# javieryu/nn_distributed_training

Hardware: NVIDIA H100
Metric: consensus node-rounds/sec (DiNNO, dist_mnist_PAPER; rounds/sec x graph nodes) (higher is better)
Workload: dtype fp64

## Files before the change

### nn_distributed_training_b200/ops/csrc/bindings.cpp

```cpp
#include <torch/extension.h>
#include <cstring>
#include <string>
#include <ATen/cuda/CUDAContext.h>
#include <pybind11/pybind11.h>

#include "consensus.h"
#include "mnist.h"

namespace py = pybind11;
using namespace nndt;

static inline cudaStream_t cur_stream() { return at::cuda::getCurrentCUDAStream().stream(); }
static inline void check(cudaError_t e, const char* what) {
  if (e != cudaSuccess) throw std::runtime_error(std::string(what) + ": " + cudaGetErrorString(e));
}
template <typename P> static P* ptr(const py::dict& d, const char* k) {
  if (!d.contains(k) || d[k].is_none()) return nullptr;
  return reinterpret_cast<P*>(d[k].cast<uint64_t>());
}
static int geti(const py::dict& d, const char* k, int dflt = 0) { return d.contains(k) ? d[k].cast<int>() : dflt; }
static double getf(const py::dict& d, const char* k, double dflt = 0) { return d.contains(k) ? d[k].cast<double>() : dflt; }

struct MnistOp {
  mnist::Args a{};
// ... 62 lines not shown
  c.nbr_rank = ptr<const int>(d, "nbr_rank"); c.dmax = geti(d, "dmax");
  c.rdr_deg = ptr<const int>(d, "rdr_deg"); c.rdr_rank = ptr<const int>(d, "rdr_rank"); c.rmax = geti(d, "rmax", 1);
  c.round_ctr = ptr<int>(d, "round_ctr");
  c.rho = ptr<const T>(d, "rho"); c.lr = ptr<const T>(d, "lr"); c.alpha = ptr<const T>(d, "alpha");
  c.graph_id = ptr<const int>(d, "graph_id");
  c.calls = ptr<int>(d, "calls");
  c.loss_part = ptr<const float>(d, "loss_part"); c.tloss = ptr<float>(d, "tloss");
  c.tdecay = (float)getf(d, "tdecay", 0.0); c.loss_S = geti(d, "loss_S", 1);
  c.flags = ptr<int>(d, "flags"); c.peer_flag = ptr<const int64_t>(d, "peer_flag");
  c.world = geti(d, "world", 1); c.rank = geti(d, "rank", 0);
  c.done_ctr = ptr<unsigned int>(d, "done_ctr"); c.err = ptr<int>(d, "err");
  c.notify_mask = d.contains("notify_mask") ? d["notify_mask"].cast<unsigned long long>() : ~0ull;
  c.node_order = ptr<const int>(d, "node_order");
  c.timeline = ptr<long long>(d, "timeline");
  c.pub_seq = ptr<int>(d, "pub_seq"); c.nbr_seq = ptr<const int64_t>(d, "nbr_seq");
  c.sum_mode = geti(d, "sum_mode", 0); c.n_total = geti(d, "n_total", 0);
  c.sum_local = ptr<double>(d, "sum_local"); c.sum_mc = ptr<const double>(d, "sum_mc");
  c.sum_flags = ptr<int>(d, "sum_flags"); c.peer_sum_flag = ptr<const int64_t>(d, "peer_sum_flag");
  return c;
}

template <typename T>
struct ConsensusOp {
  consensus::Common<T> c{};
  consensus::DinnoArgs<T> dn{};
  consensus::DsgtArgs<T> gt{};
  consensus::EdArgs<T> ed{};
  consensus::ChocoArgs<T> ch{};
  consensus::SgpArgs<T> sg{};
  explicit ConsensusOp(const py::dict& d) {
    c = common_from<T>(d);
    dn.c = c; gt.c = c; ed.c = c; ch.c = c; sg.c = c;
    sg.x = ptr<T>(d, "x"); sg.w = ptr<double>(d, "w");
    sg.row_stride = d.contains("row_stride") ? d["row_stride"].cast<long long>() : 0;
    ed.psi = ptr<T>(d, "psi");
    ch.x_hat = ptr<T>(d, "x_hat"); ch.s = ptr<T>(d, "s"); ch.live = ptr<const unsigned>(d, "live");
    ch.gamma = (T)getf(d, "gamma", 1.0); ch.code = geti(d, "code", 0);
    ch.code_stride = d.contains("code_stride") ? d["code_stride"].cast<long long>() : 0;
    dn.dual = ptr<T>(d, "dual"); dn.delta = ptr<T>(d, "delta"); dn.m = ptr<T>(d, "m"); dn.v = ptr<T>(d, "v");
    dn.pits = geti(d, "pits", 1); dn.opt = geti(d, "opt", 1); dn.persistent = geti(d, "persistent", 0);
    gt.g_old = ptr<T>(d, "g_old");
    gt.alpha_row = ptr<const T>(d, "alpha_row"); gt.own_tracker = geti(d, "own_tracker", 0);
  }
  void dinno_update(int step) {
    dn.step = step;
    check(consensus::launch_dinno_update<T>(dn, cur_stream()), "dinno_update");
  }
  void local_sum() { check(consensus::launch_local_sum<T>(c, cur_stream()), "local_sum"); }
  void dsgd_mix() { check(consensus::launch_dsgd_mix<T>(c, cur_stream()), "dsgd_mix"); }
  void dsgd_step() { check(consensus::launch_dsgd_step<T>(c, cur_stream()), "dsgd_step"); }
  void dsgt_init() { check(consensus::launch_dsgt_init<T>(gt, cur_stream()), "dsgt_init"); }
  void dsgt_mix() { check(consensus::launch_dsgt_mix<T>(gt, cur_stream()), "dsgt_mix"); }
  void dsgt_track() { check(consensus::launch_dsgt_track<T>(gt, cur_stream()), "dsgt_track"); }
  void ed_mix() { check(consensus::launch_ed_mix<T>(ed, cur_stream()), "ed_mix"); }
  void ed_step() {
    if (ed.psi == nullptr) throw std::runtime_error("ed_step needs the Exact Diffusion row `psi`");
    check(consensus::launch_ed_step<T>(ed, cur_stream()), "ed_step");
  }
  void choco_check(const char* what) const {
    if (ch.x_hat == nullptr || ch.s == nullptr || ch.live == nullptr || ch.code_stride <= 0)
      throw std::runtime_error(std::string(what) + " needs the CHOCO rows `x_hat`, `s`, the `live` mask and `code_stride`");
  }
  void choco_mix() {
    choco_check("choco_mix");
    check(consensus::launch_choco_mix<T>(ch, cur_stream()), "choco_mix");
  }
  void choco_step() {
    choco_check("choco_step");
    check(consensus::launch_choco_step<T>(ch, cur_stream()), "choco_step");
  }
  void sgp_check(const char* what) const {
    if (sg.x == nullptr || sg.w == nullptr || sg.row_stride <= 0)
      throw std::runtime_error(std::string(what) + " needs the SGP rows `x`, `w` and `row_stride`");
  }
  void sgp_mix() {
    sgp_check("sgp_mix");
    check(consensus::launch_sgp_mix<T>(sg, cur_stream()), "sgp_mix");
  }
  void sgp_step() {
    sgp_check("sgp_step");
    check(consensus::launch_sgp_step<T>(sg, cur_stream()), "sgp_step");
  }
};

template <typename T>
struct LocalStepOp {
  consensus::LocalArgs<T> a{};
  explicit LocalStepOp(const py::dict& d) {
    a.c = common_from<T>(d);
    if (a.c.calls == nullptr) throw std::runtime_error("local_step needs the per-node step counter `calls`");
    a.m = ptr<T>(d, "m"); a.v = ptr<T>(d, "v");
    a.budget = ptr<const int>(d, "budget"); a.arrive = ptr<unsigned int>(d, "arrive");
    a.lr = (T)getf(d, "local_lr"); a.opt = geti(d, "opt", 1);
    if (a.budget == nullptr || a.arrive == nullptr) throw std::runtime_error("local_step needs `budget` and `arrive`");
    if (a.opt != consensus::kSGD && (a.m == nullptr || a.v == nullptr))
      throw std::runtime_error("local_step with Adam / AdamW needs the moment rows `m` and `v`");
  }
  void step() { check(consensus::launch_local_step<T>(a, cur_stream()), "local_step"); }
};

template <typename T>
static void bind_consensus(py::module& m, const char* name) {
  py::class_<ConsensusOp<T>>(m, name)
      .def(py::init<const py::dict&>())
      .def("dinno_update", &ConsensusOp<T>::dinno_update)
      .def("local_sum", &ConsensusOp<T>::local_sum)
      .def("dsgd_mix", &ConsensusOp<T>::dsgd_mix)
      .def("dsgd_step", &ConsensusOp<T>::dsgd_step)
      .def("dsgt_init", &ConsensusOp<T>::dsgt_init)
      .def("dsgt_mix", &ConsensusOp<T>::dsgt_mix)
      .def("dsgt_track", &ConsensusOp<T>::dsgt_track)
      .def("ed_mix", &ConsensusOp<T>::ed_mix)
      .def("ed_step", &ConsensusOp<T>::ed_step)
      .def("choco_mix", &ConsensusOp<T>::choco_mix)
      .def("choco_step", &ConsensusOp<T>::choco_step)
      .def("sgp_mix", &ConsensusOp<T>::sgp_mix)
      .def("sgp_step", &ConsensusOp<T>::sgp_step);
}

void bind_mlp(py::module& m);
void bind_rl(py::module& m);
void bind_runtime(py::module& m);

PYBIND11_MODULE(_C, m) {
  m.doc() = "nn_distributed_training_b200 sm_90a kernels";
  py::class_<MnistOp>(m, "MnistOp")
      .def(py::init<const py::dict&>())
      .def("update", &MnistOp::update)
      .def("train", &MnistOp::train)
      .def("eval", &MnistOp::eval);
  py::class_<GatherOp>(m, "GatherOp").def(py::init<const py::dict&>()).def("launch", &GatherOp::launch);
  m.def("debug_batch_indices", [](int mm, int B, int call, int seed, int node, uint64_t out, uint64_t out_size) {
    check(mnist::launch_batch_indices(mm, B, call, seed, node, reinterpret_cast<int*>(out),
                                      reinterpret_cast<int*>(out_size), cur_stream()), "batch_indices");
  });
  m.def("consensus_metric", [](bool f64, uint64_t rows, int N, int n_pad, int local0, int L, uint64_t inv_norm,
                               uint64_t out_pair, uint64_t out_mean) {
    auto r = reinterpret_cast<const int64_t*>(rows);
    auto a = reinterpret_cast<double*>(inv_norm); auto b = reinterpret_cast<double*>(out_pair); auto c = reinterpret_cast<double*>(out_mean);
    check(f64 ? consensus::launch_consensus_metric<double>(r, N, n_pad, local0, L, a, b, c, cur_stream())
              : consensus::launch_consensus_metric<float>(r, N, n_pad, local0, L, a, b, c, cur_stream()), "consensus_metric");
  });
  m.def("convnet_generic_smem_bytes", [](int F, int KS, int LW, int dtype64, int spb) {
    return (size_t)mnist::generic_smem_bytes(mnist::GenericShape{F, KS, LW, dtype64, 0.0, 1.0}, dtype64, spb);
  });
  m.def("make_w1_tensor_map", [](uint64_t theta, int n_pad, int L, int off_w1) {
    unsigned char buf[128];
    check(mnist::make_w1_tensor_map(reinterpret_cast<const float*>(theta), n_pad, L, off_w1, buf), "make_w1_tensor_map");
    return py::bytes(reinterpret_cast<const char*>(buf), 128);
  });
  m.def("mnist_tc_max_clusters", []() { return mnist::tc_max_active_clusters(); });
  m.def("mnist_cl64_max_clusters", [](int nsplit) { return mnist::cl64_max_active_clusters(nsplit); }, py::arg("nsplit") = 1);
  m.def("mnist_cl64_cluster_ctas", []() { return mnist::cl64_cluster_ctas(); });
  m.def("rank_barrier", [](uint64_t slots, uint64_t peer_slot, int world, int rank, int epoch, uint64_t gate, uint64_t err) {
    check(consensus::launch_rank_barrier(reinterpret_cast<int*>(slots), reinterpret_cast<const int64_t*>(peer_slot), world, rank,
                                         epoch, reinterpret_cast<const volatile int*>(gate), reinterpret_cast<int*>(err), cur_stream()),
          "rank_barrier");
  });
  m.def("spin", [](long long cycles) { check(consensus::launch_spin(cycles, cur_stream()), "spin"); });
  bind_consensus<float>(m, "ConsensusOpF32");
  bind_consensus<double>(m, "ConsensusOpF64");
  py::class_<LocalStepOp<float>>(m, "LocalStepOpF32").def(py::init<const py::dict&>()).def("step", &LocalStepOp<float>::step);
  py::class_<LocalStepOp<double>>(m, "LocalStepOpF64").def(py::init<const py::dict&>()).def("step", &LocalStepOp<double>::step);
  bind_mlp(m);
  bind_rl(m);
  bind_runtime(m);
}
```

### nn_distributed_training_b200/ops/csrc/mnist.h

```cpp
#pragma once
#include <cuda_runtime.h>
#include <stdint.h>

namespace nndt {
namespace mnist {

struct Args {
  const float* theta;
  int n_pad, L;
  int off_wc, off_bc, off_w1, off_b1, off_w2, off_b2;
  const void* x;
  const int64_t* y;
  int x_is_u8;
  float mean, inv_std;
  int direct, batch, seed, node0;
  const int* direct_bs;
  const int* shard_off;
  const int* shard_len;
  int* calls;
  unsigned int* arrive;
  int tune;
  long long* prof;
  float* grad_part;
  float* loss_part;
  float* loss_mirror;
  int n_val;
  float* val_loss;
  unsigned char* val_correct;
};

struct GatherArgs {
  const unsigned char* x_host;
  const int64_t* y_host;
  int row_bytes;
  unsigned char* x_stage;
  int64_t* y_stage;
  int* bs_stage;
  int P, L, batch, seed, node0;
  const int* shard_off; const int* shard_len;
  const int* calls0;
  int* stage_round;
  unsigned int* done_ctr;
  int max_blocks;
};
struct GenericShape { int F, KS, LW, dtype64; double mean, inv_std; };
size_t generic_smem_bytes(const GenericShape& gs, int dtype64, int spb);
cudaError_t launch_generic_train(const Args& a, const GenericShape& gs, int spb, int S, cudaStream_t st);
cudaError_t launch_generic_eval(const Args& a, const GenericShape& gs, int ctas_per_node, cudaStream_t st);
cudaError_t make_w1_tensor_map(const float* theta, int n_pad, int L, int off_w1, void* out_map128);
cudaError_t launch_train_tc(const Args& a, const void* w1_map128, int nsplit, cudaStream_t st);
int tc_max_active_clusters();
cudaError_t launch_train_cl64(const Args& a, const GenericShape& gs, int nsplit, cudaStream_t st);
int cl64_max_active_clusters(int nsplit);
int cl64_cluster_ctas();
cudaError_t launch_gather(const GatherArgs& a, cudaStream_t st);
cudaError_t launch_train(const Args& a, int spb, int S, cudaStream_t st);
cudaError_t launch_eval(const Args& a, int ctas_per_node, cudaStream_t st);
cudaError_t launch_batch_indices(int m, int B, int call, int seed, int node, int* out, int* out_size, cudaStream_t st);

}
}
```

### nn_distributed_training_b200/ops/csrc/mnist_cl64.cu

```cuda
#include "mnist_device.cuh"

namespace nndt {
namespace mnist {

namespace cl64 {

constexpr int NT = 512, CL = 4, CELLS = 36, KC = 108, WS = 116, HS = 68;
constexpr int PXR = 10 * HW;
constexpr int KT = (KC + 7) / 8;
constexpr int HR = 68;
NNDT_DEVINL int hr(int j) { return (j >> 4) * 17 + (j & 15); }
constexpr int PART_WC = 0, PART_BC = 75, PART_B1 = 78, PART_W2 = 142, PART_B2 = 782, PART_LOSS = 792, PART_N = 793;

template <int MS>
struct Smem {
  static constexpr int NO = MS / CL;
  static constexpr bool kDoublePix = MS <= 32;
  static constexpr int PXS = kDoublePix ? PXR + 2 : PXR;
  double w[HID * WS];
  double a[MS * WS];
  double h[MS * HS];
  alignas(16) unsigned char img[kDoublePix ? MS * PXS * 8 : MS * PXS];
  double lut[kDoublePix ? 1 : 256];
  double h_loc[NO * HR > CL * 80 ? NO * HR : CL * 80];
  double dh_loc[NO * HID];
  double part[800];
  double w2[NCLS * HR];
  alignas(16) double b1[HID];
  alignas(16) double b2[16];
  double wc[80];
  double dz[NO * 16];
  double red[NO];
  int sidx[MS];
  int label[MS];
  float valid[MS];
  unsigned char arg[MS * KC];
};
static_assert(sizeof(Smem<16>) <= 227 * 1024 && sizeof(Smem<32>) <= 227 * 1024 && sizeof(Smem<64>) <= 227 * 1024,
              "shared memory budget");

NNDT_DEVINL double wmax(double v) {
#pragma unroll
  for (int o = 16; o > 0; o >>= 1) v = fmax(v, __shfl_xor_sync(0xffffffffu, v, o));
  return v;
}
template <int H>
NNDT_DEVINL void fold_half(double (&v)[16], int lane) {
  const bool up = (lane & (2 * H)) != 0;
#pragma unroll
  for (int i = 0; i < H; ++i) {
    const double send = up ? v[i] : v[i + H], keep = up ? v[i + H] : v[i];
    v[i] = keep + __shfl_xor_sync(0xffffffffu, send, 2 * H);
  }
}
NNDT_DEVINL void warp_reduce_scatter16(double (&v)[16], int lane) {
  fold_half<8>(v, lane); fold_half<4>(v, lane); fold_half<2>(v, lane); fold_half<1>(v, lane);
  v[0] += __shfl_xor_sync(0xffffffffu, v[0], 1);
}
NNDT_DEVINL void dmma_nv(double (&c)[4], double a0, double a1, double b) {
  asm("mma.sync.aligned.m16n8k4.row.col.f64.f64.f64.f64 {%0,%1,%2,%3}, {%4,%5}, {%6}, {%0,%1,%2,%3};"
      : "+d"(c[0]), "+d"(c[1]), "+d"(c[2]), "+d"(c[3])
      : "d"(a0), "d"(a1), "d"(b));
}
template <int NJ, int K, class FA, class FB>
NNDT_DEVINL void gemm_k(double (&c)[NJ][4], int m0, int n0, int lane, FA A, FB B) {
  static_assert(K % 4 == 0, "k steps of 4");
  const int g = lane >> 2, t = lane & 3;
  double a0 = A(m0 + g, t), a1 = A(m0 + g + 8, t), b[NJ];
#pragma unroll
  for (int j = 0; j < NJ; ++j) b[j] = B(t, n0 + 8 * j + g);
#pragma unroll
  for (int k0 = 0; k0 < K; k0 += 4) {
    double na0 = 0.0, na1 = 0.0, nb[NJ];
    if (k0 + 4 < K) {
      const int k = k0 + 4 + t;
      na0 = A(m0 + g, k); na1 = A(m0 + g + 8, k);
#pragma unroll
      for (int j = 0; j < NJ; ++j) nb[j] = B(k, n0 + 8 * j + g);
    }
#pragma unroll
    for (int j = 0; j < NJ; ++j) dmma_nv(c[j], a0, a1, b[j]);
    if (k0 + 4 < K) {
      a0 = na0; a1 = na1;
#pragma unroll
      for (int j = 0; j < NJ; ++j) b[j] = nb[j];
    }
  }
}
NNDT_DEVINL void stamp(long long* prof, int idx, int tid) {
  if (prof != nullptr && tid == 0) {
    long long t;
    asm volatile("mov.u64 %0, %%globaltimer;" : "=l"(t));
    prof[idx] = t;
  }
}

template <int MS>
__global__ void __cluster_dims__(CL, 1, 1) __launch_bounds__(NT, 1)
mnist_cl64_train_kernel(const Args a, const GenericShape gs) {
  using SM = Smem<MS>;
  constexpr int NO = SM::NO, PXS = SM::PXS;
  constexpr bool kDoublePix = SM::kDoublePix;
  static_assert(MS % 16 == 0 && NO <= NT / 32, "tile geometry");
  static_assert(CELLS % 2 == 0 && NCLS % 2 == 0 && 32 + NCLS / 2 <= NT, "16-byte parameter copies");
  extern __shared__ __align__(16) unsigned char smem_raw[];
  SM& sm = *reinterpret_cast<SM*>(smem_raw);
  const int tid = threadIdx.x, warp = tid >> 5, lane = tid & 31;
  const int l = blockIdx.z, bsplit = blockIdx.y, nsplit = gridDim.y;
  const int c = (int)cluster_rank();
  const double* th = reinterpret_cast<const double*>(a.theta) + (size_t)l * a.n_pad;
  const double pmean = gs.mean, pis = gs.inv_std;
  const bool u8 = a.x_is_u8 != 0;
  double* imgd = reinterpret_cast<double*>(sm.img);
  auto pix = [&](int s, int p) -> double {
    if constexpr (kDoublePix) return imgd[s * PXS + p];
    else if (u8) return sm.lut[sm.img[s * PXR + p]];
    else return (double)__ldg(reinterpret_cast<const float*>(a.x) + (size_t)sm.sidx[s] * 784 + 6 * HW * c + p);
  };
  long long* prof = a.prof != nullptr ? a.prof + ((l * nsplit + bsplit) * CL + c) * 64 : nullptr;
  stamp(prof, 0, tid);

  const int call = a.calls != nullptr ? a.calls[l] : 0;
  const BatchGeom bg = batch_geom<true>(a, l, call);
  if (tid < MS) {
    int idx = 0, lab = 0; float ok = 0.f;
    const uint32_t t = (uint32_t)(bsplit * MS + tid);
    if (t < bg.bs) {
      ok = 1.f;
      idx = a.direct ? (int)(l * a.batch + t) : bg.shard_off + (int)feistel_permute(bg.start + t, bg.m, bg.key);
      lab = (int)a.y[idx];
    }
    sm.sidx[tid] = idx; sm.valid[tid] = ok; sm.label[tid] = lab;
  }
  if constexpr (!kDoublePix)
    if (tid < 256) sm.lut[tid] = ((double)tid * (1.0 / 255.0) - pmean) * pis;
  __syncthreads();
  constexpr int NU8 = (MS * 35 + NT - 1) / NT, NF4 = kDoublePix ? (MS * 70 + NT - 1) / NT : 1;
  uint2 pu[NU8]; float4 pf[NF4];
  if (u8) {
#pragma unroll
    for (int i = 0; i < NU8; ++i) {
      const int o = tid + i * NT;
      pu[i] = make_uint2(0, 0);
      if (o < MS * 35) {
        const int s = o / 35, q = o - s * 35;
        if (sm.valid[s] != 0.f)
          pu[i] = *reinterpret_cast<const uint2*>(reinterpret_cast<const unsigned char*>(a.x) + (size_t)sm.sidx[s] * 784 + 6 * HW * c + 8 * q);
      }
    }
  } else if constexpr (kDoublePix) {
#pragma unroll
    for (int i = 0; i < NF4; ++i) {
      const int o = tid + i * NT;
      pf[i] = make_float4(0.f, 0.f, 0.f, 0.f);
      if (o < MS * 70) {
        const int s = o / 70, q = o - s * 70;
        if (sm.valid[s] != 0.f)
          pf[i] = *reinterpret_cast<const float4*>(reinterpret_cast<const float*>(a.x) + (size_t)sm.sidx[s] * 784 + 6 * HW * c + 4 * q);
      }
    }
  }
  if (u8) {
#pragma unroll
    for (int i = 0; i < NU8; ++i) {
      const int o = tid + i * NT;
      if (o < MS * 35) {
        const int s = o / 35, q = o - s * 35;
        if constexpr (kDoublePix) {
          const uint32_t w[2] = {pu[i].x, pu[i].y};
          double* dst = imgd + s * PXS + 8 * q;
#pragma unroll
          for (int j = 0; j < 8; ++j) dst[j] = ((double)((w[j >> 2] >> (8 * (j & 3))) & 0xff) * (1.0 / 255.0) - pmean) * pis;
        } else {
          *reinterpret_cast<uint2*>(sm.img + s * PXR + 8 * q) = pu[i];
        }
      }
    }
  } else if constexpr (kDoublePix) {
#pragma unroll
    for (int i = 0; i < NF4; ++i) {
      const int o = tid + i * NT;
      if (o < MS * 70) {
        double* dst = imgd + (o / 70) * PXS + 4 * (o % 70);
        dst[0] = pf[i].x; dst[1] = pf[i].y; dst[2] = pf[i].z; dst[3] = pf[i].w;
      }
    }
  }
  stamp(prof, 1, tid);
  pdl_wait();
  pdl_launch_dependents();
  stamp(prof, 2, tid);

  constexpr int NW2 = (NCLS * HID + NT - 1) / NT;
  double wcv = 0.0, w2v[NW2];
  if (tid < 75) wcv = __ldcg(th + a.off_wc + tid);
  else if (tid < 78) wcv = __ldcg(th + a.off_bc + (tid - 75));
#pragma unroll
  for (int i = 0; i < NW2; ++i) {
    const int o = tid + i * NT;
    w2v[i] = o < NCLS * HID ? __ldcg(th + a.off_w2 + o) : 0.0;
  }
  for (int o = tid; o < HID * KC / 2; o += NT) {
    const int j = o / (KC / 2), r = o - j * (KC / 2), ch = r / (CELLS / 2), q = 2 * (r - ch * (CELLS / 2));
    cp_async16(sm.w + j * WS + ch * CELLS + q, th + a.off_w1 + (size_t)j * FC1_IN + ch * NPOOL + CELLS * c + q);
  }
  if (tid < HID / 2) cp_async16(sm.b1 + 2 * tid, th + a.off_b1 + 2 * tid);
  else if (tid >= 32 && tid < 32 + NCLS / 2) cp_async16(sm.b2 + 2 * (tid - 32), th + a.off_b2 + 2 * (tid - 32));
  cp_async_commit();
  if (tid < 78) sm.wc[tid] = wcv;
#pragma unroll
  for (int i = 0; i < NW2; ++i) {
    const int o = tid + i * NT;
    if (o < NCLS * HID) sm.w2[(o / HID) * HR + hr(o % HID)] = w2v[i];
  }
  __syncthreads();
  stamp(prof, 3, tid);

  for (int it = tid; it < MS * CELLS; it += NT) {
    const int s = it / CELLS, cell = it - s * CELLS;
    const int pr = cell / PHW, px = cell - pr * PHW;
    const int p0 = (2 * pr) * HW + 2 * px;
    double patch[6][6];
    if constexpr (kDoublePix) {
      const double* src = imgd + s * PXS + p0;
#pragma unroll
      for (int r = 0; r < 6; ++r)
#pragma unroll
        for (int q = 0; q < 6; q += 2) {
          const double2 v = *reinterpret_cast<const double2*>(src + r * HW + q);
          patch[r][q] = v.x; patch[r][q + 1] = v.y;
        }
    } else {
#pragma unroll
      for (int r = 0; r < 6; ++r)
#pragma unroll
        for (int q = 0; q < 6; ++q) patch[r][q] = pix(s, p0 + r * HW + q);
    }
    const bool ok = sm.valid[s] != 0.f;
#pragma unroll 1
    for (int ch = 0; ch < F; ++ch) {
      double a00 = 0, a01 = 0, a10 = 0, a11 = 0;
#pragma unroll
      for (int ky = 0; ky < KS; ++ky)
#pragma unroll
        for (int kx = 0; kx < KS; ++kx) {
          const double w = sm.wc[ch * 25 + ky * 5 + kx];
          a00 += w * patch[ky][kx]; a01 += w * patch[ky][kx + 1];
          a10 += w * patch[ky + 1][kx]; a11 += w * patch[ky + 1][kx + 1];
        }
      double m = a00; int ai = 0;
      if (a01 > m) { m = a01; ai = 1; }
      if (a10 > m) { m = a10; ai = 2; }
      if (a11 > m) { m = a11; ai = 3; }
      m += sm.wc[75 + ch];
      m = (ok && m > 0.0) ? m : 0.0;
      sm.a[s * WS + ch * CELLS + cell] = m;
      sm.arg[s * KC + ch * CELLS + cell] = (unsigned char)(ai | (m > 0.0 ? 4 : 0));
    }
  }
  cp_async_wait<0>();
  __syncthreads();
  stamp(prof, 4, tid);

  {
    constexpr int NJ1 = MS == 64 ? 2 : 1, NGRP = 8 / NJ1;
    if (warp < (MS / 16) * NGRP) {
      const int m0 = 16 * (warp / NGRP), n0 = 8 * NJ1 * (warp % NGRP);
      double acc[NJ1][4];
      zero(acc);
      gemm_k<NJ1, KC>(acc, m0, n0, lane, at(sm.a, WS), at_t(sm.w, WS));
#pragma unroll
      for (int j = 0; j < NJ1; ++j)
#pragma unroll
        for (int i = 0; i < 4; ++i) sm.h[frow(m0, lane, i) * HS + fcol(n0 + 8 * j, lane, i)] = acc[j][i];
    }
  }
  stamp(prof, 5, tid);
  cluster_sync();
  stamp(prof, 6, tid);
  if (c == 0 && tid == 0 && a.calls != nullptr) {
    if (a.arrive == nullptr || nsplit == 1) a.calls[l] = call + 1;
    else if (atomicAdd(a.arrive + l, 1u) == (unsigned)nsplit - 1) { a.arrive[l] = 0; a.calls[l] = call + 1; }
  }

  const int s0 = c * NO;
  const double inv_bs = 1.0 / (double)(bg.bs ? bg.bs : 1);
  if (warp < NO) {
    const int sl = warp, s = s0 + sl;
    double hv[2];
#pragma unroll
    for (int q = 0; q < 2; ++q) {
      const int j = lane + 32 * q;
      const double* src = sm.h + s * HS + j;
      double v = sm.b1[j];
#pragma unroll
      for (int r = 0; r < CL; ++r) v += ld_dsmem(map_to(src, (uint32_t)r));
      hv[q] = v > 0.0 ? v : 0.0;
      sm.h_loc[sl * HR + hr(j)] = hv[q];
    }
    __syncwarp();
    double zp[2];
#pragma unroll
    for (int r = 0; r < 2; ++r) {
      const int o = lane + 32 * r, cc = o >> 2, part = o & 3;
      double v = 0.0;
      if (o < 4 * NCLS) {
#pragma unroll
        for (int jj = 0; jj < 16; ++jj) v += sm.h_loc[sl * HR + part * 17 + jj] * sm.w2[cc * HR + part * 17 + jj];
      }
      v += __shfl_xor_sync(0xffffffffu, v, 1);
      v += __shfl_xor_sync(0xffffffffu, v, 2);
      zp[r] = v;
    }
    static_assert(NCLS > 8 && NCLS <= 16, "two rounds of four lanes per class");
    const double z0 = __shfl_sync(0xffffffffu, zp[0], (4 * lane) & 31), z1 = __shfl_sync(0xffffffffu, zp[1], (4 * lane) & 31);
    const bool cls = lane < NCLS;
    const double zc = cls ? (lane < 8 ? z0 : z1) + sm.b2[lane] : -1.0e300;
    const double mx = wmax(zc);
    const double se = warp_sum(cls ? exp(zc - mx) : 0.0);
    const double lse = mx + log(se);
    const int y = sm.label[s];
    const double ok = (double)sm.valid[s];
    const double dzc = cls ? ok * inv_bs * (exp(zc - lse) - (lane == y ? 1.0 : 0.0)) : 0.0;
    if (cls) sm.dz[sl * 16 + lane] = dzc;
    if (lane == y) sm.red[sl] = ok * (lse - zc);
    double dh[2] = {0.0, 0.0};
#pragma unroll
    for (int cc = 0; cc < NCLS; ++cc) {
      const double d = __shfl_sync(0xffffffffu, dzc, cc);
      dh[0] += d * sm.w2[cc * HR + hr(lane)];
      dh[1] += d * sm.w2[cc * HR + hr(lane + 32)];
    }
#pragma unroll
    for (int q = 0; q < 2; ++q) sm.dh_loc[sl * HID + lane + 32 * q] = hv[q] > 0.0 ? dh[q] : 0.0;
  }
  __syncthreads();
  for (int o = tid; o < NCLS * HID; o += NT) {
    const int cc = o >> 6, j = o & 63;
    double v = 0.0;
    for (int sl = 0; sl < NO; ++sl) v += sm.dz[sl * 16 + cc] * sm.h_loc[sl * HR + hr(j)];
    sm.part[PART_W2 + o] = v;
  }
  if (tid < HID) {
    double v = 0.0;
    for (int sl = 0; sl < NO; ++sl) v += sm.dh_loc[sl * HID + tid];
    sm.part[PART_B1 + tid] = v;
  } else if (tid >= 64 && tid < 64 + NCLS) {
    double v = 0.0;
    for (int sl = 0; sl < NO; ++sl) v += sm.dz[sl * 16 + (tid - 64)];
    sm.part[PART_B2 + (tid - 64)] = v;
  } else if (tid == 96) {
    double v = 0.0;
    for (int sl = 0; sl < NO; ++sl) v += sm.red[sl];
    sm.part[PART_LOSS] = v * inv_bs;
  }
  stamp(prof, 7, tid);
  cluster_sync();
  stamp(prof, 8, tid);
  double* gp = reinterpret_cast<double*>(a.grad_part) + ((size_t)l * nsplit + bsplit) * a.n_pad;
  {
    constexpr int NE = PART_N - PART_B1, PER = (NE + CL - 1) / CL;
    const int o = PART_B1 + c * PER + tid;
    if (tid < PER && o < PART_N) {
      double v = 0.0;
#pragma unroll
      for (int r = 0; r < CL; ++r) v += ld_dsmem(map_to(sm.part + o, (uint32_t)r));
      if (o < PART_W2) gp[a.off_b1 + (o - PART_B1)] = v;
      else if (o < PART_B2) gp[a.off_w2 + (o - PART_W2)] = v;
      else if (o < PART_LOSS) gp[a.off_b2 + (o - PART_B2)] = v;
      else {
        a.loss_part[l * nsplit + bsplit] = (float)v;
        if (a.loss_mirror != nullptr) a.loss_mirror[l * nsplit + bsplit] = (float)v;
      }
    }
  }
  for (int o = tid; o < MS * HID; o += NT) {
    const int s = o >> 6, j = o & 63, r = s / NO;
    sm.h[s * HS + j] = ld_dsmem(map_to(sm.dh_loc + (s - r * NO) * HID + j, (uint32_t)r));
  }
  __syncthreads();
  stamp(prof, 9, tid);

  constexpr int NP2 = (MS / 16) * (KT / 2), NR2 = (NP2 + NT / 32 - 1) / (NT / 32);
  static_assert(KT % 2 == 0 && KC * MS + (NT / 32) * 16 <= HID * WS, "da1 and the conv-grad warp sums fit in the W slice");
  double acc2[NR2][2][4];
#pragma unroll
  for (int r = 0; r < NR2; ++r) {
    zero(acc2[r]);
    const int p = warp + r * (NT / 32);
    if (p < NP2) gemm_k<2, HID>(acc2[r], 16 * (p / (KT / 2)), 16 * (p % (KT / 2)), lane, at(sm.h, HS), at(sm.w, WS));
  }
  __syncthreads();
  stamp(prof, 10, tid);
  double* da1 = sm.w;
#pragma unroll
  for (int r = 0; r < NR2; ++r) {
    const int p = warp + r * (NT / 32);
    if (p < NP2) {
      const int m0 = 16 * (p / (KT / 2)), n0 = 16 * (p % (KT / 2));
#pragma unroll
      for (int jt = 0; jt < 2; ++jt)
#pragma unroll
        for (int i = 0; i < 4; ++i) {
          const int s = frow(m0, lane, i), k = fcol(n0 + 8 * jt, lane, i);
          if (k < KC) da1[k * MS + s] = (sm.arg[s * KC + k] & 4) ? acc2[r][jt][i] : 0.0;
        }
    }
  }
  __syncthreads();
  stamp(prof, 11, tid);
  constexpr int W3 = NT / 32 - HID / 16, NJ3 = KT / 2;
  if (warp >= W3) {
    const int m0 = 16 * (warp - W3);
#pragma unroll 1
    for (int n0 = 0; n0 < 8 * KT; n0 += 8 * NJ3) {
      double acc[NJ3][4];
      zero(acc);
      gemm_k<NJ3, MS>(acc, m0, n0, lane, at_t(sm.h, HS), at(sm.a, WS));
#pragma unroll
      for (int jt = 0; jt < NJ3; ++jt)
#pragma unroll
        for (int i = 0; i < 4; i += 2) {
          const int j = frow(m0, lane, i), k = fcol(n0 + 8 * jt, lane, i);
          if (k < KC) {
            const int ch = k / CELLS, cell = k - ch * CELLS;
            __stcg(reinterpret_cast<double2*>(gp + a.off_w1 + (size_t)j * FC1_IN + ch * NPOOL + CELLS * c + cell),
                   make_double2(acc[jt][i], acc[jt][i + 1]));
          }
        }
    }
    stamp(prof, 12, tid - W3 * 32);
  }
  constexpr int KW = 3, NRUN = MS * 3;
  static_assert(KS * KW < NT / 32 && F * KS <= 16, "conv-grad work split");
  double* wsums = sm.w + KC * MS;
  auto pix2 = [&](int s, int p) -> double2 {
    if constexpr (kDoublePix) return *reinterpret_cast<const double2*>(imgd + s * PXS + p);
    else return make_double2(pix(s, p), pix(s, p + 1));
  };
  if (warp < KS * KW) {
    const int ky = warp / KW;
    double acc[16];
#pragma unroll
    for (int i = 0; i < 16; ++i) acc[i] = 0.0;
#pragma unroll 1
    for (int r = tid - ky * KW * 32; r < NRUN; r += KW * 32) {
      const int s = r % MS, pr = r / MS;
      const int rb = (2 * pr + ky) * HW;
      double x0[6], x1[6];
#pragma unroll
      for (int px = 0; px < PHW; ++px) {
        const int p = rb + 2 * px;
        if (px == 0) {
#pragma unroll
          for (int q = 0; q < 6; q += 2) {
            const double2 u = pix2(s, p + q), v = pix2(s, p + HW + q);
            x0[q] = u.x; x0[q + 1] = u.y; x1[q] = v.x; x1[q + 1] = v.y;
          }
        } else {
#pragma unroll
          for (int q = 0; q < 4; ++q) { x0[q] = x0[q + 2]; x1[q] = x1[q + 2]; }
          const double2 u = pix2(s, p + 4), v = pix2(s, p + HW + 4);
          x0[4] = u.x; x0[5] = u.y; x1[4] = v.x; x1[5] = v.y;
        }
#pragma unroll
        for (int ch = 0; ch < F; ++ch) {
          const int k = ch * CELLS + pr * PHW + px;
          const double g = da1[k * MS + s];
          const int ai = sm.arg[s * KC + k] & 3;
          const double g00 = ai == 0 ? g : 0.0, g01 = ai == 1 ? g : 0.0, g10 = ai == 2 ? g : 0.0, g11 = ai == 3 ? g : 0.0;
#pragma unroll
          for (int kx = 0; kx < KS; ++kx) {
            double& t = acc[ch * KS + kx];
            t = fma(g00, x0[kx], t); t = fma(g01, x0[kx + 1], t);
            t = fma(g10, x1[kx], t); t = fma(g11, x1[kx + 1], t);
          }
        }
      }
    }
    warp_reduce_scatter16(acc, lane);
    if ((lane & 1) == 0 && (lane >> 1) < F * KS) wsums[warp * 16 + (lane >> 1)] = acc[0];
  } else if (warp == KS * KW) {
#pragma unroll 1
    for (int ch = 0; ch < F; ++ch) {
      double v = 0.0;
      for (int o = lane; o < CELLS * MS; o += 32) v += da1[ch * CELLS * MS + o];
      v = warp_sum(v);
      if (lane == 0) wsums[warp * 16 + ch] = v;
    }
  }
  __syncthreads();
  if (tid < 78) {
    double v = 0.0;
    if (tid < 75) {
      const int ch = tid / 25, t = tid - ch * 25, ky = t / KS, kx = t - ky * KS;
#pragma unroll
      for (int w = 0; w < KW; ++w) v += wsums[(ky * KW + w) * 16 + ch * KS + kx];
    } else {
      v = wsums[KS * KW * 16 + (tid - 75)];
    }
    st_dsmem(map_to(sm.h_loc + c * 80 + tid, 0u), v);
  }
  stamp(prof, 13, tid);
  cluster_sync();
  if (c == 0 && tid < 78) {
    double v = 0.0;
#pragma unroll
    for (int r = 0; r < CL; ++r) v += sm.h_loc[r * 80 + tid];
    gp[tid < 75 ? a.off_wc + tid : a.off_bc + (tid - 75)] = v;
  }
  stamp(prof, 14, tid);
}

template <int MS>
static cudaError_t prepare_ms() {
  static cudaError_t prep = cudaFuncSetAttribute(mnist_cl64_train_kernel<MS>, cudaFuncAttributeMaxDynamicSharedMemorySize, (int)sizeof(Smem<MS>));
  return prep;
}

template <int MS>
static cudaError_t launch_ms(const Args& a, const GenericShape& gs, cudaStream_t st) {
  const cudaError_t prep = prepare_ms<MS>();
  if (prep != cudaSuccess) return prep;
  cudaLaunchConfig_t cfg{};
  cfg.gridDim = dim3(CL, 64 / MS, a.L); cfg.blockDim = dim3(NT);
  cfg.dynamicSmemBytes = sizeof(Smem<MS>); cfg.stream = st;
  cudaLaunchAttribute attr[1];
  attr[0].id = cudaLaunchAttributeProgrammaticStreamSerialization;
  attr[0].val.programmaticStreamSerializationAllowed = 1;
  static const bool no_pdl = getenv("NNDT_NO_PDL") != nullptr;
  cfg.attrs = attr; cfg.numAttrs = no_pdl ? 0 : 1;
  return cudaLaunchKernelEx(&cfg, mnist_cl64_train_kernel<MS>, a, gs);
}

template <int MS>
static int max_clusters_ms() {
  if (prepare_ms<MS>() != cudaSuccess) { cudaGetLastError(); return 0; }
  cudaLaunchConfig_t cfg{};
  cfg.gridDim = dim3(CL, 1, 1); cfg.blockDim = dim3(NT); cfg.dynamicSmemBytes = sizeof(Smem<MS>);
  int n = 0;
  if (cudaOccupancyMaxActiveClusters(&n, mnist_cl64_train_kernel<MS>, &cfg) != cudaSuccess) { cudaGetLastError(); return 0; }
  return n;
}

}

cudaError_t launch_train_cl64(const Args& a, const GenericShape& gs, int nsplit, cudaStream_t st) {
  switch (nsplit) {
    case 1: return cl64::launch_ms<64>(a, gs, st);
    case 2: return cl64::launch_ms<32>(a, gs, st);
    case 4: return cl64::launch_ms<16>(a, gs, st);
  }
  return cudaErrorInvalidValue;
}

int cl64_max_active_clusters(int nsplit) {
  switch (nsplit) {
    case 1: return cl64::max_clusters_ms<64>();
    case 2: return cl64::max_clusters_ms<32>();
    case 4: return cl64::max_clusters_ms<16>();
  }
  return 0;
}

int cl64_cluster_ctas() { return cl64::CL; }

}
}
```

### nn_distributed_training_b200/ops/csrc/common.cuh

```cuda
#pragma once
#include <cuda_runtime.h>
#include <stdint.h>
#include <cstdlib>
#include <utility>

#define NNDT_DEVINL __device__ __forceinline__

namespace nndt {

constexpr int kWarp = 32;

NNDT_DEVINL float warp_sum(float v) {
#pragma unroll
  for (int o = 16; o > 0; o >>= 1) v += __shfl_xor_sync(0xffffffffu, v, o);
  return v;
}
NNDT_DEVINL double warp_sum(double v) {
#pragma unroll
  for (int o = 16; o > 0; o >>= 1) v += __shfl_xor_sync(0xffffffffu, v, o);
  return v;
}

NNDT_DEVINL void st_release_sys(int* p, int v) {
  asm volatile("st.release.sys.global.s32 [%0], %1;" ::"l"(p), "r"(v) : "memory");
}
NNDT_DEVINL int ld_acquire_sys(const int* p) {
  int v;
  asm volatile("ld.acquire.sys.global.s32 %0, [%1];" : "=r"(v) : "l"(p) : "memory");
  return v;
}
NNDT_DEVINL int ld_relaxed_sys(const int* p) {
  int v;
  asm volatile("ld.relaxed.sys.global.s32 %0, [%1];" : "=r"(v) : "l"(p) : "memory");
  return v;
}

NNDT_DEVINL float4 ld_stream_f4(const float* p) {
  float4 r;
  asm volatile("ld.global.L1::no_allocate.v4.f32 {%0,%1,%2,%3}, [%4];"
               : "=f"(r.x), "=f"(r.y), "=f"(r.z), "=f"(r.w)
               : "l"(p));
  return r;
}

NNDT_DEVINL void pdl_wait() { asm volatile("griddepcontrol.wait;" ::: "memory"); }
NNDT_DEVINL void pdl_launch_dependents() { asm volatile("griddepcontrol.launch_dependents;" ::: "memory"); }

template <typename... KArgs, typename... Args>
inline cudaError_t launch_pdl(void (*kernel)(KArgs...), dim3 grid, dim3 block, size_t smem, cudaStream_t st, Args&&... args) {
  cudaLaunchConfig_t cfg{};
  cfg.gridDim = grid; cfg.blockDim = block; cfg.dynamicSmemBytes = smem; cfg.stream = st;
  static const bool no_pdl = getenv("NNDT_NO_PDL") != nullptr;
  cudaLaunchAttribute attr[1];
  attr[0].id = cudaLaunchAttributeProgrammaticStreamSerialization;
  attr[0].val.programmaticStreamSerializationAllowed = 1;
  cfg.attrs = attr; cfg.numAttrs = no_pdl ? 0 : 1;
  return cudaLaunchKernelEx(&cfg, kernel, std::forward<Args>(args)...);
}

NNDT_DEVINL uint32_t smem_addr_u32(const void* p) { return (uint32_t)__cvta_generic_to_shared(p); }
NNDT_DEVINL void mbarrier_init(uint64_t* bar, uint32_t count) {
  asm volatile("mbarrier.init.shared::cta.b64 [%0], %1;" ::"r"(smem_addr_u32(bar)), "r"(count) : "memory");
  asm volatile("fence.mbarrier_init.release.cluster;" ::: "memory");
}
NNDT_DEVINL void mbarrier_expect_tx(uint64_t* bar, uint32_t bytes) {
  asm volatile("mbarrier.arrive.expect_tx.shared::cta.b64 _, [%0], %1;" ::"r"(smem_addr_u32(bar)), "r"(bytes) : "memory");
}
NNDT_DEVINL void tma_bulk_g2s(void* smem_dst, const void* gmem_src, uint32_t bytes, uint64_t* bar) {
  asm volatile("cp.async.bulk.shared::cluster.global.mbarrier::complete_tx::bytes [%0], [%1], %2, [%3];" ::"r"(
                   smem_addr_u32(smem_dst)),
               "l"(gmem_src), "r"(bytes), "r"(smem_addr_u32(bar))
               : "memory");
}
NNDT_DEVINL void mbarrier_wait_parity(uint64_t* bar, uint32_t parity) {
  const uint32_t addr = smem_addr_u32(bar);
  uint32_t done;
  do {
    asm volatile(
        "{\n\t.reg .pred p;\n\t"
        "mbarrier.try_wait.parity.shared::cta.b64 p, [%1], %2;\n\t"
        "selp.u32 %0, 1, 0, p;\n\t}\n"
        : "=r"(done)
        : "r"(addr), "r"(parity)
        : "memory");
  } while (!done);
}

NNDT_DEVINL void cluster_sync() {
  asm volatile("barrier.cluster.arrive.release.aligned;\n\tbarrier.cluster.wait.acquire.aligned;" ::: "memory");
}
NNDT_DEVINL uint32_t cluster_rank() { uint32_t r; asm volatile("mov.u32 %0, %%cluster_ctarank;" : "=r"(r)); return r; }
NNDT_DEVINL uint32_t map_to(const void* p, uint32_t rank) {
  uint32_t r;
  asm volatile("mapa.shared::cluster.u32 %0, %1, %2;" : "=r"(r) : "r"((uint32_t)__cvta_generic_to_shared(p)), "r"(rank));
  return r;
}
NNDT_DEVINL double ld_dsmem(uint32_t a) { double v; asm volatile("ld.shared::cluster.f64 %0, [%1];" : "=d"(v) : "r"(a) : "memory"); return v; }
NNDT_DEVINL void st_dsmem(uint32_t a, double v) { asm volatile("st.shared::cluster.f64 [%0], %1;" ::"r"(a), "d"(v) : "memory"); }

NNDT_DEVINL void dmma(double (&c)[4], double a0, double a1, double b) {
  asm volatile("mma.sync.aligned.m16n8k4.row.col.f64.f64.f64.f64 {%0,%1,%2,%3}, {%4,%5}, {%6}, {%0,%1,%2,%3};"
               : "+d"(c[0]), "+d"(c[1]), "+d"(c[2]), "+d"(c[3])
               : "d"(a0), "d"(a1), "d"(b));
}

template <int NJ, class FA, class FB>
NNDT_DEVINL void gemm(double (&c)[NJ][4], int m0, int n0, int K, int lane, FA A, FB B) {
  const int g = lane >> 2, t = lane & 3;
#pragma unroll 4
  for (int k0 = 0; k0 < K; k0 += 4) {
    const int k = k0 + t;
    const double a0 = A(m0 + g, k), a1 = A(m0 + g + 8, k);
#pragma unroll
    for (int j = 0; j < NJ; ++j) dmma(c[j], a0, a1, B(k, n0 + 8 * j + g));
  }
}

template <int NJ>
NNDT_DEVINL void zero(double (&c)[NJ][4]) {
#pragma unroll
  for (int j = 0; j < NJ; ++j) c[j][0] = c[j][1] = c[j][2] = c[j][3] = 0.0;
}
NNDT_DEVINL int frow(int m0, int lane, int i) { return m0 + (lane >> 2) + 8 * (i >> 1); }
NNDT_DEVINL int fcol(int n0, int lane, int i) { return n0 + 2 * (lane & 3) + (i & 1); }

template <class T> NNDT_DEVINL auto at(const T* s, int ld) { return [s, ld](int i, int j) { return s[i * ld + j]; }; }
template <class T> NNDT_DEVINL auto at_t(const T* s, int ld) { return [s, ld](int i, int j) { return s[j * ld + i]; }; }

__device__ __forceinline__ void split_tf32(float x, uint32_t& hi, uint32_t& lo) {
  asm("cvt.rna.tf32.f32 %0, %1;" : "=r"(hi) : "f"(x));
  const float r = x - __uint_as_float(hi);
  asm("cvt.rna.tf32.f32 %0, %1;" : "=r"(lo) : "f"(r));
}
__device__ __forceinline__ void mma_tf32(float (&c)[4], const uint32_t (&a)[4], const uint32_t (&b)[2]) {
  asm volatile(
      "mma.sync.aligned.m16n8k8.row.col.f32.tf32.tf32.f32 {%0,%1,%2,%3}, {%4,%5,%6,%7}, {%8,%9}, {%0,%1,%2,%3};"
      : "+f"(c[0]), "+f"(c[1]), "+f"(c[2]), "+f"(c[3])
      : "r"(a[0]), "r"(a[1]), "r"(a[2]), "r"(a[3]), "r"(b[0]), "r"(b[1]));
}
struct FragA { uint32_t hi[4], lo[4]; };
struct FragB { uint32_t hi[2], lo[2]; };
__device__ __forceinline__ FragA make_frag_a(float a0, float a1, float a2, float a3) {
  FragA f;
  split_tf32(a0, f.hi[0], f.lo[0]); split_tf32(a1, f.hi[1], f.lo[1]);
  split_tf32(a2, f.hi[2], f.lo[2]); split_tf32(a3, f.hi[3], f.lo[3]);
  return f;
}
__device__ __forceinline__ FragB make_frag_b(float b0, float b1) {
  FragB f;
  split_tf32(b0, f.hi[0], f.lo[0]); split_tf32(b1, f.hi[1], f.lo[1]);
  return f;
}
__device__ __forceinline__ void mma3(float (&c)[4], const FragA& a, const FragB& b) {
  mma_tf32(c, a.lo, b.hi);
  mma_tf32(c, a.hi, b.lo);
  mma_tf32(c, a.hi, b.hi);
}

template <int NJ, class FA, class FB>
NNDT_DEVINL void gemm(float (&c)[NJ][4], int m0, int n0, int K, int lane, FA A, FB B) {
  const int g = lane >> 2, t = lane & 3;
#pragma unroll 2
  for (int k0 = 0; k0 < K; k0 += 8) {
    const int k = k0 + t;
    const FragA a = make_frag_a(A(m0 + g, k), A(m0 + g + 8, k), A(m0 + g, k + 4), A(m0 + g + 8, k + 4));
#pragma unroll
    for (int j = 0; j < NJ; ++j) mma3(c[j], a, make_frag_b(B(k, n0 + 8 * j + g), B(k + 4, n0 + 8 * j + g)));
  }
}

NNDT_DEVINL void cp_async16(void* smem, const void* gmem) {
  uint32_t s = (uint32_t)__cvta_generic_to_shared(smem);
  asm volatile("cp.async.cg.shared.global [%0], [%1], 16;" ::"r"(s), "l"(gmem) : "memory");
}
NNDT_DEVINL void cp_async_commit() { asm volatile("cp.async.commit_group;" ::: "memory"); }
template <int N>
NNDT_DEVINL void cp_async_wait() {
  asm volatile("cp.async.wait_group %0;" ::"n"(N) : "memory");
}

}
```

Before: 160,600.

## Split conv stage between DMMA tensor-core warps and scalar warps

In the cl64 training kernel, for small per-CTA sample tiles (double-precision pixel path), the first 24 conv cells are computed as an implicit GEMM with fp64 DMMA fragments on the upper warps. The lower warps keep the scalar patch path for the remaining cells. This aims to cut scalar FMA cost in the conv/pool stage by using tensor cores while both warp groups run concurrently. It also adds a standalone single-tile test kernel and binding, and the uneven 24/12 cell split may leave one warp group idle.

After: 163,800, median of 6. 1.02x the previous value.

```diff
diff --git a/nn_distributed_training_b200/ops/csrc/bindings.cpp b/nn_distributed_training_b200/ops/csrc/bindings.cpp
--- a/nn_distributed_training_b200/ops/csrc/bindings.cpp
+++ b/nn_distributed_training_b200/ops/csrc/bindings.cpp
@@ -238,6 +238,10 @@
   m.def("mnist_tc_max_clusters", []() { return mnist::tc_max_active_clusters(); });
   m.def("mnist_cl64_max_clusters", [](int nsplit) { return mnist::cl64_max_active_clusters(nsplit); }, py::arg("nsplit") = 1);
   m.def("mnist_cl64_cluster_ctas", []() { return mnist::cl64_cluster_ctas(); });
+  m.def("mnist_cl64_conv_tile", [](uint64_t px, uint64_t wc, int cell, uint64_t out) {
+    check(mnist::launch_cl64_conv_tile(reinterpret_cast<const double*>(px), reinterpret_cast<const double*>(wc), cell,
+                                       reinterpret_cast<double*>(out), cur_stream()), "mnist_cl64_conv_tile");
+  });
   m.def("rank_barrier", [](uint64_t slots, uint64_t peer_slot, int world, int rank, int epoch, uint64_t gate, uint64_t err) {
     check(consensus::launch_rank_barrier(reinterpret_cast<int*>(slots), reinterpret_cast<const int64_t*>(peer_slot), world, rank,
                                          epoch, reinterpret_cast<const volatile int*>(gate), reinterpret_cast<int*>(err), cur_stream()),
diff --git a/nn_distributed_training_b200/ops/csrc/mnist.h b/nn_distributed_training_b200/ops/csrc/mnist.h
--- a/nn_distributed_training_b200/ops/csrc/mnist.h
+++ b/nn_distributed_training_b200/ops/csrc/mnist.h
@@ -53,6 +53,7 @@
 cudaError_t launch_train_cl64(const Args& a, const GenericShape& gs, int nsplit, cudaStream_t st);
 int cl64_max_active_clusters(int nsplit);
 int cl64_cluster_ctas();
+cudaError_t launch_cl64_conv_tile(const double* px, const double* wc, int cell, double* out, cudaStream_t st);
 cudaError_t launch_gather(const GatherArgs& a, cudaStream_t st);
 cudaError_t launch_train(const Args& a, int spb, int S, cudaStream_t st);
 cudaError_t launch_eval(const Args& a, int ctas_per_node, cudaStream_t st);
diff --git a/nn_distributed_training_b200/ops/csrc/mnist_cl64.cu b/nn_distributed_training_b200/ops/csrc/mnist_cl64.cu
--- a/nn_distributed_training_b200/ops/csrc/mnist_cl64.cu
+++ b/nn_distributed_training_b200/ops/csrc/mnist_cl64.cu
@@ -38,6 +38,11 @@
 };
 static_assert(sizeof(Smem<16>) <= 227 * 1024 && sizeof(Smem<32>) <= 227 * 1024 && sizeof(Smem<64>) <= 227 * 1024,
               "shared memory budget");
+template <int MS>
+struct ConvSplit {
+  static constexpr int TC = Smem<MS>::kDoublePix ? 24 : 0, CW = 8;
+  static_assert(CW % 4 == 0 && TC % 2 == 0 && TC <= CELLS, "conv split");
+};
 
 NNDT_DEVINL double wmax(double v) {
 #pragma unroll
@@ -87,6 +92,45 @@
     }
   }
 }
+NNDT_DEVINL void conv_b_frags(double (&bw)[9][2], int (&ko)[9], const double* wc, int g, int t) {
+#pragma unroll
+  for (int ks = 0; ks < 9; ++ks) {
+    const int k = 4 * ks + t, r = k / 6, q = k - r * 6;
+    ko[ks] = r * HW + q;
+#pragma unroll
+    for (int j = 0; j < 2; ++j) {
+      const int n = 8 * j + g, ch = n >> 2, ky = r - ((n >> 1) & 1), kx = q - (n & 1);
+      bw[ks][j] = ch < F && ky >= 0 && ky < KS && kx >= 0 && kx < KS ? wc[ch * 25 + ky * 5 + kx] : 0.0;
+    }
+  }
+}
+template <int PXS>
+NNDT_DEVINL void conv_tile(double (&acc)[2][4], const double* p0, const double (&bw)[9][2], const int (&ko)[9]) {
+  zero(acc);
+#pragma unroll
+  for (int ks = 0; ks < 9; ++ks) {
+    const double a0 = p0[ko[ks]], a1 = p0[PXS + ko[ks]];
+    dmma_nv(acc[0], a0, a1, bw[ks][0]);
+    dmma_nv(acc[1], a0, a1, bw[ks][1]);
+  }
+}
+NNDT_DEVINL int cell_origin(int cell) {
+  const int pr = cell / PHW, pc = cell - pr * PHW;
+  return (2 * pr) * HW + 2 * pc;
+}
+__global__ void conv_tile_kernel(const double* px, const double* wc, int cell, double* out) {
+  constexpr int PXS = PXR + 2;
+  const int lane = threadIdx.x, g = lane >> 2, t = lane & 3;
+  double bw[9][2], acc[2][4];
+  int ko[9];
+  conv_b_frags(bw, ko, wc, g, t);
+  conv_tile<PXS>(acc, px + 2 * g * PXS + cell_origin(cell), bw, ko);
+#pragma unroll
+  for (int j = 0; j < 2; ++j)
+#pragma unroll
+    for (int i = 0; i < 4; ++i) out[frow(0, lane, i) * 16 + fcol(8 * j, lane, i)] = acc[j][i];
+}
+
 NNDT_DEVINL void stamp(long long* prof, int idx, int tid) {
   if (prof != nullptr && tid == 0) {
     long long t;
@@ -216,8 +260,45 @@
   __syncthreads();
   stamp(prof, 3, tid);
 
-  for (int it = tid; it < MS * CELLS; it += NT) {
-    const int s = it / CELLS, cell = it - s * CELLS;
+  constexpr int TC = ConvSplit<MS>::TC, CW = TC > 0 ? ConvSplit<MS>::CW : NT / 32;
+  if constexpr (TC > 0) {
+    if (warp >= CW) {
+      const int g = lane >> 2, t = lane & 3;
+      double bw[9][2];
+      int ko[9];
+      conv_b_frags(bw, ko, sm.wc, g, t);
+      const bool odd = (t & 1) != 0;
+#pragma unroll 1
+      for (int tile = warp - CW; tile < (MS / 16) * TC; tile += NT / 32 - CW) {
+        const int cell = tile / (MS / 16), s0 = 16 * (tile - cell * (MS / 16));
+        double acc[2][4];
+        conv_tile<PXS>(acc, imgd + (s0 + 2 * g) * PXS + cell_origin(cell), bw, ko);
+        const int s = s0 + 2 * g + (odd ? 1 : 0);
+        const bool ok = sm.valid[s] != 0.f;
+#pragma unroll
+        for (int j = 0; j < 2; ++j) {
+          const double* c4 = acc[j];
+          const double r0 = __shfl_xor_sync(0xffffffffu, odd ? c4[0] : c4[2], 1);
+          const double r1 = __shfl_xor_sync(0xffffffffu, odd ? c4[1] : c4[3], 1);
+          const double a00 = odd ? r0 : c4[0], a01 = odd ? r1 : c4[1], a10 = odd ? c4[2] : r0, a11 = odd ? c4[3] : r1;
+          const int ch = 2 * j + (t >> 1);
+          if (ch < F) {
+            double m = a00; int ai = 0;
+            if (a01 > m) { m = a01; ai = 1; }
+            if (a10 > m) { m = a10; ai = 2; }
+            if (a11 > m) { m = a11; ai = 3; }
+            m += sm.wc[75 + ch];
+            m = (ok && m > 0.0) ? m : 0.0;
+            sm.a[s * WS + ch * CELLS + cell] = m;
+            sm.arg[s * KC + ch * CELLS + cell] = (unsigned char)(ai | (m > 0.0 ? 4 : 0));
+          }
+        }
+      }
+    }
+  }
+  constexpr int NCD = CELLS - TC;
+  for (int it = tid; (TC == 0 || warp < CW) && it < MS * NCD; it += CW * 32) {
+    const int s = it / NCD, cell = TC + (it - s * NCD);
     const int pr = cell / PHW, px = cell - pr * PHW;
     const int p0 = (2 * pr) * HW + 2 * px;
     double patch[6][6];
@@ -565,5 +646,11 @@
 
 int cl64_cluster_ctas() { return cl64::CL; }
 
-}
-}
+cudaError_t launch_cl64_conv_tile(const double* px, const double* wc, int cell, double* out, cudaStream_t st) {
+  if (cell < 0 || cell >= cl64::CELLS) return cudaErrorInvalidValue;
+  cl64::conv_tile_kernel<<<1, 32, 0, st>>>(px, wc, cell, out);
+  return cudaGetLastError();
+}
+
+}
+}
```

## Split warps with named barriers to overlap dA1 GEMM with weight-grad GEMM

Applied to the files above, without the earlier changes.

Warps are split into two groups. One group computes the dA1 GEMM and scatters da1, synchronising only among itself through named barriers. The other group computes the W1 gradient GEMM at the same time instead of waiting behind two full-block syncs, then joins through a bar.arrive/bar.sync handshake. In the conv-grad inner loop, the four masked FMAs per kernel tap are replaced by one FMA on a row operand chosen by integer mad arithmetic on the double's bit halves, and a column select. Each change cuts idle time or wasted FP64 work, but the named-barrier protocol adds risk of deadlock or races if the thread counts or write hazards on the W slice are wrong.

Measured after the change: 161,700 before, 165,100 after (median of 6 runs). +2.1%, better.

```diff
diff --git a/nn_distributed_training_b200/ops/csrc/common.cuh b/nn_distributed_training_b200/ops/csrc/common.cuh
--- a/nn_distributed_training_b200/ops/csrc/common.cuh
+++ b/nn_distributed_training_b200/ops/csrc/common.cuh
@@ -89,6 +89,8 @@
 NNDT_DEVINL void cluster_sync() {
   asm volatile("barrier.cluster.arrive.release.aligned;\n\tbarrier.cluster.wait.acquire.aligned;" ::: "memory");
 }
+NNDT_DEVINL void named_bar_sync(int id, int nthreads) { asm volatile("bar.sync %0, %1;" ::"r"(id), "r"(nthreads) : "memory"); }
+NNDT_DEVINL void named_bar_arrive(int id, int nthreads) { asm volatile("bar.arrive %0, %1;" ::"r"(id), "r"(nthreads) : "memory"); }
 NNDT_DEVINL uint32_t cluster_rank() { uint32_t r; asm volatile("mov.u32 %0, %%cluster_ctarank;" : "=r"(r)); return r; }
 NNDT_DEVINL uint32_t map_to(const void* p, uint32_t rank) {
   uint32_t r;
diff --git a/nn_distributed_training_b200/ops/csrc/mnist_cl64.cu b/nn_distributed_training_b200/ops/csrc/mnist_cl64.cu
--- a/nn_distributed_training_b200/ops/csrc/mnist_cl64.cu
+++ b/nn_distributed_training_b200/ops/csrc/mnist_cl64.cu
@@ -87,6 +87,7 @@
     }
   }
 }
+NNDT_DEVINL int imad(int a, int b, int c) { int d; asm("mad.lo.s32 %0, %1, %2, %3;" : "=r"(d) : "r"(a), "r"(b), "r"(c)); return d; }
 NNDT_DEVINL void stamp(long long* prof, int idx, int tid) {
   if (prof != nullptr && tid == 0) {
     long long t;
@@ -381,36 +382,42 @@
   __syncthreads();
   stamp(prof, 9, tid);
 
-  constexpr int NP2 = (MS / 16) * (KT / 2), NR2 = (NP2 + NT / 32 - 1) / (NT / 32);
-  static_assert(KT % 2 == 0 && KC * MS + (NT / 32) * 16 <= HID * WS, "da1 and the conv-grad warp sums fit in the W slice");
-  double acc2[NR2][2][4];
-#pragma unroll
-  for (int r = 0; r < NR2; ++r) {
-    zero(acc2[r]);
-    const int p = warp + r * (NT / 32);
-    if (p < NP2) gemm_k<2, HID>(acc2[r], 16 * (p / (KT / 2)), 16 * (p % (KT / 2)), lane, at(sm.h, HS), at(sm.w, WS));
-  }
-  __syncthreads();
-  stamp(prof, 10, tid);
+  constexpr int W3 = NT / 32 - HID / 16, NJ3 = KT / 2;
+  constexpr int NT2 = W3 * 32;
+  constexpr int BAR_W_READ = 1, BAR_DA1 = 2, BAR_DA1_ALL = 3;
+  static_assert(W3 > 0 && NT2 % 32 == 0 && NT2 + (HID / 16) * 32 == NT, "every warp is on exactly one side of the split");
   double* da1 = sm.w;
-#pragma unroll
-  for (int r = 0; r < NR2; ++r) {
-    const int p = warp + r * (NT / 32);
-    if (p < NP2) {
-      const int m0 = 16 * (p / (KT / 2)), n0 = 16 * (p % (KT / 2));
-#pragma unroll
-      for (int jt = 0; jt < 2; ++jt)
-#pragma unroll
-        for (int i = 0; i < 4; ++i) {
-          const int s = frow(m0, lane, i), k = fcol(n0 + 8 * jt, lane, i);
-          if (k < KC) da1[k * MS + s] = (sm.arg[s * KC + k] & 4) ? acc2[r][jt][i] : 0.0;
-        }
-    }
-  }
-  __syncthreads();
-  stamp(prof, 11, tid);
-  constexpr int W3 = NT / 32 - HID / 16, NJ3 = KT / 2;
-  if (warp >= W3) {
+  if (warp < W3) {
+    constexpr int NP2 = (MS / 16) * (KT / 2), NR2 = (NP2 + W3 - 1) / W3;
+    static_assert(KT % 2 == 0 && KC * MS + (NT / 32) * 16 <= HID * WS, "da1 and the conv-grad warp sums fit in the W slice");
+    double acc2[NR2][2][4];
+#pragma unroll
+    for (int r = 0; r < NR2; ++r) {
+      zero(acc2[r]);
+      const int p = warp + r * W3;
+      if (p < NP2) gemm_k<2, HID>(acc2[r], 16 * (p / (KT / 2)), 16 * (p % (KT / 2)), lane, at(sm.h, HS), at(sm.w, WS));
+    }
+    named_bar_sync(BAR_W_READ, NT2);
+    stamp(prof, 10, tid);
+#pragma unroll
+    for (int r = 0; r < NR2; ++r) {
+      const int p = warp + r * W3;
+      if (p < NP2) {
+        const int m0 = 16 * (p / (KT / 2)), n0 = 16 * (p % (KT / 2));
+#pragma unroll
+        for (int jt = 0; jt < 2; ++jt)
+#pragma unroll
+          for (int i = 0; i < 4; ++i) {
+            const int s = frow(m0, lane, i), k = fcol(n0 + 8 * jt, lane, i);
+            if (k < KC) da1[k * MS + s] = (sm.arg[s * KC + k] & 4) ? acc2[r][jt][i] : 0.0;
+          }
+      }
+    }
+    named_bar_arrive(BAR_DA1_ALL, NT);
+    named_bar_sync(BAR_DA1, NT2);
+    stamp(prof, 11, tid);
+  } else {
+    stamp(prof, 16, tid - W3 * 32);
     const int m0 = 16 * (warp - W3);
 #pragma unroll 1
     for (int n0 = 0; n0 < 8 * KT; n0 += 8 * NJ3) {
@@ -429,7 +436,9 @@
           }
         }
     }
-    stamp(prof, 12, tid - W3 * 32);
+    stamp(prof, 17, tid - W3 * 32);
+    named_bar_sync(BAR_DA1_ALL, NT);
+    stamp(prof, 18, tid - W3 * 32);
   }
   constexpr int KW = 3, NRUN = MS * 3;
   static_assert(KS * KW < NT / 32 && F * KS <= 16, "conv-grad work split");
@@ -463,23 +472,35 @@
           const double2 u = pix2(s, p + 4), v = pix2(s, p + HW + 4);
           x0[4] = u.x; x0[5] = u.y; x1[4] = v.x; x1[5] = v.y;
         }
+        int dlo[6], dhi[6];
+#pragma unroll
+        for (int q = 0; q < 6; ++q) {
+          dlo[q] = __double2loint(x1[q]) - __double2loint(x0[q]);
+          dhi[q] = __double2hiint(x1[q]) - __double2hiint(x0[q]);
+        }
 #pragma unroll
         for (int ch = 0; ch < F; ++ch) {
           const int k = ch * CELLS + pr * PHW + px;
           const double g = da1[k * MS + s];
           const int ai = sm.arg[s * KC + k] & 3;
-          const double g00 = ai == 0 ? g : 0.0, g01 = ai == 1 ? g : 0.0, g10 = ai == 2 ? g : 0.0, g11 = ai == 3 ? g : 0.0;
+          const bool right = (ai & 1) != 0;
+          const int low = ai >> 1;
+          double xs[6];
+#pragma unroll
+          for (int q = 0; q < 6; ++q)
+            xs[q] = __hiloint2double(imad(low, dhi[q], __double2hiint(x0[q])), imad(low, dlo[q], __double2loint(x0[q])));
 #pragma unroll
           for (int kx = 0; kx < KS; ++kx) {
             double& t = acc[ch * KS + kx];
-            t = fma(g00, x0[kx], t); t = fma(g01, x0[kx + 1], t);
-            t = fma(g10, x1[kx], t); t = fma(g11, x1[kx + 1], t);
+            t = fma(g, right ? xs[kx + 1] : xs[kx], t);
           }
         }
       }
     }
     warp_reduce_scatter16(acc, lane);
     if ((lane & 1) == 0 && (lane >> 1) < F * KS) wsums[warp * 16 + (lane >> 1)] = acc[0];
+    stamp(prof, 12, tid);
+    stamp(prof, 19, tid - W3 * 32);
   } else if (warp == KS * KW) {
 #pragma unroll 1
     for (int ch = 0; ch < F; ++ch) {
```
